# apple/ml-quant

Measured on AMD Instinct MI355X. Metric: images/sec ResNet-18 LS-1w/LS-2a 224x224 eval forward, higher is better.
Workload: dtype fp4 (e2m1, unit block scales) mfma on sign bits: exact integers in the f32 accumulator + f32; 1 GPU; ResNet-18 ImageNet ls-1 weight / ls-2 activation, synthetic 3x224x224, batch 256 per GPU, random-init weights; global_batch=256, parallelism=dp1 (batch-sharded replicas, RCCL all-gather of logits)

## Files before the change

### ml-quant_amd/csrc/lsq_pointwise.hip

```cpp

#include "lsq_common.h"

#ifdef LSQ_PW_SYNCTHREADS
#define PW_BARRIER() __syncthreads()
#else
#define PW_BARRIER() lds_barrier()
#endif
namespace lsq {
namespace {

typedef __attribute__((ext_vector_type(16))) float f32x16;

struct PwArgs {
  const float* x;
  const float* w;
  const float* bias;
  float* y;
  int N, C, H, W, O, Ho, Wo, s;
  long long P;
};

constexpr int kPitch = 68;

__global__ __launch_bounds__(256) void pointwise_conv_kernel(PwArgs a) {
  __shared__ __attribute__((aligned(16))) float ws[64][kPitch];
  __shared__ __attribute__((aligned(16))) float xs[64][kPitch];
  const int tid = threadIdx.x, lane = tid & 63, wid = tid >> 6;
  const unsigned n_ot = (unsigned)a.O >> 6;
  const long long p0 = (long long)(blockIdx.x / n_ot) * 64;
  const int o0 = (int)(blockIdx.x % n_ot) * 64;
  const int HoWo = a.Ho * a.Wo;
  const long long HW = (long long)a.H * a.W;
  const long long sp = min(p0 + lane, a.P - 1);
  const int sn = (int)(sp / HoWo);
  const int sr = (int)(sp - (long long)sn * HoWo);
  const int sho = sr / a.Wo, swo = sr - sho * a.Wo;
  const unsigned xoff = (unsigned)(((long long)sn * a.C + 16 * wid) * HW + (long long)sho * a.s * a.W + swo * a.s);
  const float* __restrict__ xsrc = a.x;
  const unsigned woff = (unsigned)(16 * wid * a.C + lane);
  const float* __restrict__ wsrc = a.w + (long long)o0 * a.C;
  const int mt = wid >> 1, nt = wid & 1;
  const int col = lane & 31, g = lane >> 5;
  f32x16 acc = {};
  float xv[16], wv[16];
#pragma unroll
  for (int i = 0; i < 16; ++i) xv[i] = (xsrc + (long long)i * HW)[xoff];
#pragma unroll
  for (int i = 0; i < 16; ++i) wv[i] = (wsrc + (long long)i * a.C)[woff];
  for (int c0 = 0; c0 < a.C; c0 += 64) {
    __syncthreads();
#pragma unroll
    for (int q = 0; q < 4; ++q)
      *reinterpret_cast<float4*>(&xs[lane][16 * wid + 4 * q]) = make_float4(xv[4 * q], xv[4 * q + 1], xv[4 * q + 2], xv[4 * q + 3]);
#pragma unroll
    for (int i = 0; i < 16; ++i) ws[16 * wid + i][lane] = wv[i];
    __syncthreads();
    if (c0 + 64 < a.C) {
#pragma unroll
      for (int i = 0; i < 16; ++i) xv[i] = (xsrc + (long long)(c0 + 64 + i) * HW)[xoff];
#pragma unroll
      for (int i = 0; i < 16; ++i) wv[i] = (wsrc + (long long)i * a.C + c0 + 64)[woff];
    }
#pragma unroll
    for (int h = 0; h < 2; ++h) {
      float4 af[4], bf[4];
#pragma unroll
      for (int q = 0; q < 4; ++q) {
        af[q] = *reinterpret_cast<const float4*>(&ws[mt * 32 + col][32 * g + 16 * h + 4 * q]);
        bf[q] = *reinterpret_cast<const float4*>(&xs[nt * 32 + col][32 * g + 16 * h + 4 * q]);
      }
#pragma unroll
      for (int q = 0; q < 4; ++q) {
        acc = __builtin_amdgcn_mfma_f32_32x32x2f32(af[q].x, bf[q].x, acc, 0, 0, 0);
        acc = __builtin_amdgcn_mfma_f32_32x32x2f32(af[q].y, bf[q].y, acc, 0, 0, 0);
        acc = __builtin_amdgcn_mfma_f32_32x32x2f32(af[q].z, bf[q].z, acc, 0, 0, 0);
        acc = __builtin_amdgcn_mfma_f32_32x32x2f32(af[q].w, bf[q].w, acc, 0, 0, 0);
      }
    }
  }
  const long long p = p0 + nt * 32 + col;
  const int ob = o0 + mt * 32 + 4 * g;
  float bv[16];
  if (a.bias) {
#pragma unroll
    for (int reg = 0; reg < 16; ++reg) bv[reg] = a.bias[ob + (reg & 3) + 8 * (reg >> 2)];
  } else {
#pragma unroll
    for (int reg = 0; reg < 16; ++reg) bv[reg] = 0.f;
  }
  if (p >= a.P) return;
  const int n = (int)(p / HoWo);
  const int r = (int)(p - (long long)n * HoWo);
  const unsigned yoff = (unsigned)(((long long)n * a.O + ob) * HoWo + r);
#pragma unroll
  for (int reg = 0; reg < 16; ++reg) (a.y + (long long)((reg & 3) + 8 * (reg >> 2)) * HoWo)[yoff] = acc[reg] + bv[reg];
}

typedef float f32x4 __attribute__((ext_vector_type(4)));

template <int NOT, bool PAIRS, bool VEC4>
__global__ __launch_bounds__(256) void pointwise_all_kernel(PwArgs a) {
  __shared__ __attribute__((aligned(16))) float ws[2][64][kPitch];
  __shared__ __attribute__((aligned(16))) float xs[64][kPitch];
  const int tid = threadIdx.x, lane = tid & 63, wid = tid >> 6;
  const long long p0 = (long long)blockIdx.x * 64;
  const int ob = (int)blockIdx.y * (NOT * 64);
  const int HoWo = a.Ho * a.Wo;
  const long long HW = (long long)a.H * a.W;
  const float* __restrict__ xsrc = a.x;
  unsigned xoff;
  if constexpr (PAIRS) {
    const long long sp = min(p0 + 2 * (tid & 31), a.P - 2);
    const int sn = (int)(sp / HoWo);
    const int sr = (int)(sp - (long long)sn * HoWo);
    const int sho = sr / a.Wo, swo = sr - sho * a.Wo;
    xoff = (unsigned)(((long long)sn * a.C + 8 * (tid >> 5)) * HW + (long long)sho * a.s * a.W + swo * a.s);
  } else {
    const long long sp = min(p0 + lane, a.P - 1);
    const int sn = (int)(sp / HoWo);
    const int sr = (int)(sp - (long long)sn * HoWo);
    const int sho = sr / a.Wo, swo = sr - sho * a.Wo;
    xoff = (unsigned)(((long long)sn * a.C + 16 * wid) * HW + (long long)sho * a.s * a.W + swo * a.s);
  }
  const unsigned woff = (unsigned)((tid >> 4) * a.C + 4 * (tid & 15));
  const int mt = wid >> 1, nt = wid & 1;
  const int col = lane & 31, g = lane >> 5;
  f32x16 acc[NOT];
#pragma unroll
  for (int t = 0; t < NOT; ++t)
#pragma unroll
    for (int q = 0; q < 16; ++q) acc[t][q] = 0.f;

  f32x4 xq[8];
  float xv[16];
  auto load_x = [&](int c0) {
    if constexpr (PAIRS) {
#pragma unroll
      for (int i = 0; i < 8; ++i) xq[i] = *reinterpret_cast<const f32x4*>(xsrc + (long long)(c0 + i) * HW + xoff);
    } else {
#pragma unroll
      for (int i = 0; i < 16; ++i) xv[i] = (xsrc + (long long)(c0 + i) * HW)[xoff];
    }
  };
  auto store_x = [&]() {
    if constexpr (PAIRS) {
      const int px = 2 * (tid & 31), cb = 8 * (tid >> 5);
      *reinterpret_cast<float4*>(&xs[px][cb]) = make_float4(xq[0][0], xq[1][0], xq[2][0], xq[3][0]);
      *reinterpret_cast<float4*>(&xs[px][cb + 4]) = make_float4(xq[4][0], xq[5][0], xq[6][0], xq[7][0]);
      *reinterpret_cast<float4*>(&xs[px + 1][cb]) = make_float4(xq[0][2], xq[1][2], xq[2][2], xq[3][2]);
      *reinterpret_cast<float4*>(&xs[px + 1][cb + 4]) = make_float4(xq[4][2], xq[5][2], xq[6][2], xq[7][2]);
    } else {
#pragma unroll
      for (int q = 0; q < 4; ++q)
        *reinterpret_cast<float4*>(&xs[lane][16 * wid + 4 * q]) = make_float4(xv[4 * q], xv[4 * q + 1], xv[4 * q + 2], xv[4 * q + 3]);
    }
  };
  f32x4 wq[4];
  auto load_w = [&](int t, int c0) {
    const float* wsrc = a.w + (long long)(ob + t * 64) * a.C + c0;
#pragma unroll
    for (int k = 0; k < 4; ++k) wq[k] = *reinterpret_cast<const f32x4*>(wsrc + (long long)(16 * k) * a.C + woff);
  };
  auto store_w = [&](int buf) {
#pragma unroll
    for (int k = 0; k < 4; ++k)
      *reinterpret_cast<float4*>(&ws[buf][(tid >> 4) + 16 * k][4 * (tid & 15)]) = make_float4(wq[k][0], wq[k][1], wq[k][2], wq[k][3]);
  };

  const int nchunks = a.C >> 6;
  load_x(0);
  load_w(0, 0);
  int buf = 0;
  for (int cc = 0; cc < nchunks; ++cc) {
    PW_BARRIER();
    store_x();
    if (cc + 1 < nchunks) load_x(64 * (cc + 1));
#pragma unroll
    for (int t = 0; t < NOT; ++t) {
      store_w(buf);
      PW_BARRIER();
      if (t + 1 < NOT) load_w(t + 1, 64 * cc);
      else if (cc + 1 < nchunks) load_w(0, 64 * (cc + 1));
#pragma unroll
      for (int h = 0; h < 2; ++h) {
        float4 af[4], bf[4];
#pragma unroll
        for (int q = 0; q < 4; ++q) {
          af[q] = *reinterpret_cast<const float4*>(&ws[buf][mt * 32 + col][32 * g + 16 * h + 4 * q]);
          bf[q] = *reinterpret_cast<const float4*>(&xs[nt * 32 + col][32 * g + 16 * h + 4 * q]);
        }
#pragma unroll
        for (int q = 0; q < 4; ++q) {
          acc[t] = __builtin_amdgcn_mfma_f32_32x32x2f32(bf[q].x, af[q].x, acc[t], 0, 0, 0);
          acc[t] = __builtin_amdgcn_mfma_f32_32x32x2f32(bf[q].y, af[q].y, acc[t], 0, 0, 0);
          acc[t] = __builtin_amdgcn_mfma_f32_32x32x2f32(bf[q].z, af[q].z, acc[t], 0, 0, 0);
          acc[t] = __builtin_amdgcn_mfma_f32_32x32x2f32(bf[q].w, af[q].w, acc[t], 0, 0, 0);
        }
      }
      buf ^= 1;
    }
  }
#pragma unroll
  for (int t = 0; t < NOT; ++t) {
    const int o = ob + 64 * t + mt * 32 + col;
    const float b = a.bias ? a.bias[o] : 0.f;
#pragma unroll
    for (int rg = 0; rg < 4; ++rg) {
      const long long p = p0 + nt * 32 + 8 * rg + 4 * g;
      if constexpr (VEC4) {
        if (p < a.P) {
          const int n = (int)(p / HoWo);
          const int r = (int)(p - (long long)n * HoWo);
          const f32x4 v = {acc[t][4 * rg] + b, acc[t][4 * rg + 1] + b, acc[t][4 * rg + 2] + b, acc[t][4 * rg + 3] + b};
          *reinterpret_cast<f32x4*>(a.y + ((long long)n * a.O + o) * HoWo + r) = v;
        }
      } else {
#pragma unroll
        for (int k = 0; k < 4; ++k) {
          const long long pk = p + k;
          if (pk < a.P) {
            const int n = (int)(pk / HoWo);
            const int r = (int)(pk - (long long)n * HoWo);
            a.y[((long long)n * a.O + o) * HoWo + r] = acc[t][4 * rg + k] + b;
          }
        }
      }
    }
  }
}

template <int NOT>
void launch_all(const PwArgs& a, dim3 grid, hipStream_t st) {
  const bool vec4 = ((a.Ho * a.Wo) & 3) == 0;
  if (a.s == 2 && (a.Wo & 1) == 0 && a.P >= 2) {
    if (vec4) hipLaunchKernelGGL((pointwise_all_kernel<NOT, true, true>), grid, dim3(256), 0, st, a);
    else hipLaunchKernelGGL((pointwise_all_kernel<NOT, true, false>), grid, dim3(256), 0, st, a);
  } else {
    if (vec4) hipLaunchKernelGGL((pointwise_all_kernel<NOT, false, true>), grid, dim3(256), 0, st, a);
    else hipLaunchKernelGGL((pointwise_all_kernel<NOT, false, false>), grid, dim3(256), 0, st, a);
  }
}

}
}

using namespace lsq;

extern "C" int lsq_pointwise_conv(const float* x, int N, int C, int H, int W, const float* w, const float* bias, int O,
                                  int stride, float* y, void* stream) {
  if (!x || !w || !y) return LSQ_E_NULL;
  if (N <= 0 || C <= 0 || H <= 0 || W <= 0 || O <= 0 || stride <= 0) return LSQ_E_SHAPE;
  if (C % 64 || O % 64) return LSQ_E_UNSUPPORTED;
  if ((long long)N * C * H * W >= (1ll << 30) || (long long)N * O * ((H - 1) / stride + 1) * ((W - 1) / stride + 1) >= (1ll << 30))
    return LSQ_E_UNSUPPORTED;
  PwArgs a = {};
  a.x = x; a.w = w; a.bias = bias; a.y = y;
  a.N = N; a.C = C; a.H = H; a.W = W; a.O = O; a.s = stride;
  a.Ho = (H - 1) / stride + 1;
  a.Wo = (W - 1) / stride + 1;
  a.P = (long long)N * a.Ho * a.Wo;
  const long long blocks = (a.P + 63) / 64;
  if (blocks * (O / 64) > 0x7FFFFFFF) return LSQ_E_SHAPE;
  const int n_ot = O / 64;
  const bool pair_ok = stride != 2 || (a.Wo & 1) || (W & 1) == 0;
  if (n_ot <= 8 && (n_ot & (n_ot - 1)) == 0 && pair_ok) {
    int per_wg = n_ot;
    long long min_wgs = 256;
#ifdef LSQ_TUNE
    if (const char* e = getenv("LSQ_PW_MINWG")) min_wgs = atoll(e);
#endif
    while (per_wg > 1 && blocks * (n_ot / per_wg) < min_wgs) per_wg >>= 1;
    const dim3 grid((unsigned)blocks, (unsigned)(n_ot / per_wg));
    switch (per_wg) {
      case 1: launch_all<1>(a, grid, (hipStream_t)stream); break;
      case 2: launch_all<2>(a, grid, (hipStream_t)stream); break;
      case 4: launch_all<4>(a, grid, (hipStream_t)stream); break;
      default: launch_all<8>(a, grid, (hipStream_t)stream); break;
    }
    return (int)hipGetLastError();
  }
  hipLaunchKernelGGL(pointwise_conv_kernel, dim3((unsigned)(blocks * (O / 64))), dim3(256), 0, (hipStream_t)stream, a);
  return (int)hipGetLastError();
}
```

Measured before the change: 125,000 images/sec.

## Make pointwise conv kernel persistent with double-buffered x and load-balanced tile split

Replaces the one-tile-per-workgroup pointwise (1x1) conv kernel with a persistent kernel. Each workgroup walks a contiguous range of pixel tiles, with the grid sized to 2 workgroups per CU and an optional swizzle for grouping. The x tile is now double-buffered in LDS, weights are prefetched two steps ahead and stay resident when they fit, and output-channel grouping is chosen by a wave-quantization load model. The goal is to cut launch tail and wave-quantization waste, overlap global loads with MFMA work, and drop per-tile index division. The cost is more LDS per workgroup, which lowers occupancy, plus more complex indexing and a hardcoded CU count.

```diff
diff --git a/ml-quant_amd/csrc/lsq_pointwise.hip b/ml-quant_amd/csrc/lsq_pointwise.hip
--- a/ml-quant_amd/csrc/lsq_pointwise.hip
+++ b/ml-quant_amd/csrc/lsq_pointwise.hip
@@ -1,3 +1,6 @@
+
+#include <algorithm>
+#include <type_traits>
 
 #include "lsq_common.h"
 
@@ -97,97 +100,173 @@
 }
 
 typedef float f32x4 __attribute__((ext_vector_type(4)));
-
-template <int NOT, bool PAIRS, bool VEC4>
-__global__ __launch_bounds__(256) void pointwise_all_kernel(PwArgs a) {
+typedef float f32x4u __attribute__((ext_vector_type(4), aligned(4)));
+
+constexpr int kPwCus = 256;
+constexpr int kPwWgsPerCu = 2;
+
+struct PwSplit {
+  unsigned tiles;
+  unsigned ngroups;
+  unsigned base, rem;
+  int swz;
+};
+
+template <int NOT, bool WRES, bool PAIRS>
+__global__ __launch_bounds__(256) void pointwise_persistent_kernel(PwArgs a, PwSplit sp) {
   __shared__ __attribute__((aligned(16))) float ws[2][64][kPitch];
-  __shared__ __attribute__((aligned(16))) float xs[64][kPitch];
+  __shared__ __attribute__((aligned(16))) float xs[2][64][kPitch];
   const int tid = threadIdx.x, lane = tid & 63, wid = tid >> 6;
-  const long long p0 = (long long)blockIdx.x * 64;
-  const int ob = (int)blockIdx.y * (NOT * 64);
-  const int HoWo = a.Ho * a.Wo;
-  const long long HW = (long long)a.H * a.W;
+  unsigned grp, idx;
+  if (sp.swz) {
+    const unsigned k = blockIdx.x >> 3;
+    grp = k % sp.ngroups;
+    idx = (k / sp.ngroups) * 8 + (blockIdx.x & 7);
+  } else {
+    grp = blockIdx.x % sp.ngroups;
+    idx = blockIdx.x / sp.ngroups;
+  }
+  const unsigned tile0 = idx * sp.base + min(idx, sp.rem);
+  const unsigned nu = sp.base + (idx < sp.rem ? 1u : 0u);
+  const int ob = (int)grp * (NOT * 64);
+  const unsigned P = (unsigned)a.P, HoWo = (unsigned)(a.Ho * a.Wo), HW = (unsigned)(a.H * a.W);
+  const int nchunks = a.C >> 6;
   const float* __restrict__ xsrc = a.x;
-  unsigned xoff;
-  if constexpr (PAIRS) {
-    const long long sp = min(p0 + 2 * (tid & 31), a.P - 2);
-    const int sn = (int)(sp / HoWo);
-    const int sr = (int)(sp - (long long)sn * HoWo);
-    const int sho = sr / a.Wo, swo = sr - sho * a.Wo;
-    xoff = (unsigned)(((long long)sn * a.C + 8 * (tid >> 5)) * HW + (long long)sho * a.s * a.W + swo * a.s);
-  } else {
-    const long long sp = min(p0 + lane, a.P - 1);
-    const int sn = (int)(sp / HoWo);
-    const int sr = (int)(sp - (long long)sn * HoWo);
-    const int sho = sr / a.Wo, swo = sr - sho * a.Wo;
-    xoff = (unsigned)(((long long)sn * a.C + 16 * wid) * HW + (long long)sho * a.s * a.W + swo * a.s);
-  }
-  const unsigned woff = (unsigned)((tid >> 4) * a.C + 4 * (tid & 15));
+  auto x_offset = [&](unsigned tile) __attribute__((always_inline)) -> unsigned {
+    const unsigned spx = PAIRS ? min(tile * 64 + 2 * (tid & 31), P - 2) : min(tile * 64 + lane, P - 1);
+    const unsigned sn = spx / HoWo, sr = spx - sn * HoWo;
+    const unsigned sho = sr / (unsigned)a.Wo, swo = sr - sho * (unsigned)a.Wo;
+    return ((sn * a.C + (PAIRS ? 8 * (tid >> 5) : 16 * wid)) * HW + sho * a.s * a.W + swo * a.s) * 4;
+  };
+  f32x4 xq[8];
+  float xv[16];
+  auto load_x = [&](int cc, unsigned xoff) __attribute__((always_inline)) {
+    const char* src = reinterpret_cast<const char*>(xsrc + (long long)(64 * cc) * HW);
+    if constexpr (PAIRS) {
+#pragma unroll
+      for (int i = 0; i < 8; ++i) xq[i] = *reinterpret_cast<const f32x4u*>(src + (long long)i * HW * 4 + xoff);
+    } else {
+#pragma unroll
+      for (int i = 0; i < 16; ++i) xv[i] = *reinterpret_cast<const float*>(src + (long long)i * HW * 4 + xoff);
+    }
+  };
+  auto store_x = [&](int buf) __attribute__((always_inline)) {
+    if constexpr (PAIRS) {
+      const int px = 2 * (tid & 31), cb = 8 * (tid >> 5);
+      *reinterpret_cast<float4*>(&xs[buf][px][cb]) = make_float4(xq[0][0], xq[1][0], xq[2][0], xq[3][0]);
+      *reinterpret_cast<float4*>(&xs[buf][px][cb + 4]) = make_float4(xq[4][0], xq[5][0], xq[6][0], xq[7][0]);
+      *reinterpret_cast<float4*>(&xs[buf][px + 1][cb]) = make_float4(xq[0][2], xq[1][2], xq[2][2], xq[3][2]);
+      *reinterpret_cast<float4*>(&xs[buf][px + 1][cb + 4]) = make_float4(xq[4][2], xq[5][2], xq[6][2], xq[7][2]);
+    } else {
+#pragma unroll
+      for (int q = 0; q < 4; ++q)
+        *reinterpret_cast<float4*>(&xs[buf][lane][16 * wid + 4 * q]) = make_float4(xv[4 * q], xv[4 * q + 1], xv[4 * q + 2], xv[4 * q + 3]);
+    }
+  };
+  const unsigned woff = (unsigned)((tid >> 4) * a.C + 4 * (tid & 15)) * 4;
+  const float* __restrict__ wsrc = a.w + (long long)ob * a.C;
+  f32x4 wq[2][4];
+  auto load_w = [&](f32x4 (&r)[4], int t, int cc) {
+    const char* src = reinterpret_cast<const char*>(wsrc + (long long)(t * 64) * a.C + 64 * cc);
+#pragma unroll
+    for (int k = 0; k < 4; ++k) r[k] = *reinterpret_cast<const f32x4*>(src + (long long)(16 * k) * a.C * 4 + woff);
+  };
+  auto store_w = [&](int buf, const f32x4 (&r)[4]) {
+#pragma unroll
+    for (int k = 0; k < 4; ++k)
+      *reinterpret_cast<float4*>(&ws[buf][(tid >> 4) + 16 * k][4 * (tid & 15)]) = make_float4(r[k][0], r[k][1], r[k][2], r[k][3]);
+  };
   const int mt = wid >> 1, nt = wid & 1;
   const int col = lane & 31, g = lane >> 5;
   f32x16 acc[NOT];
-#pragma unroll
-  for (int t = 0; t < NOT; ++t)
+  float bv[NOT];
+#pragma unroll
+  for (int t = 0; t < NOT; ++t) {
 #pragma unroll
     for (int q = 0; q < 16; ++q) acc[t][q] = 0.f;
-
-  f32x4 xq[8];
-  float xv[16];
-  auto load_x = [&](int c0) {
-    if constexpr (PAIRS) {
-#pragma unroll
-      for (int i = 0; i < 8; ++i) xq[i] = *reinterpret_cast<const f32x4*>(xsrc + (long long)(c0 + i) * HW + xoff);
-    } else {
-#pragma unroll
-      for (int i = 0; i < 16; ++i) xv[i] = (xsrc + (long long)(c0 + i) * HW)[xoff];
-    }
-  };
-  auto store_x = [&]() {
-    if constexpr (PAIRS) {
-      const int px = 2 * (tid & 31), cb = 8 * (tid >> 5);
-      *reinterpret_cast<float4*>(&xs[px][cb]) = make_float4(xq[0][0], xq[1][0], xq[2][0], xq[3][0]);
-      *reinterpret_cast<float4*>(&xs[px][cb + 4]) = make_float4(xq[4][0], xq[5][0], xq[6][0], xq[7][0]);
-      *reinterpret_cast<float4*>(&xs[px + 1][cb]) = make_float4(xq[0][2], xq[1][2], xq[2][2], xq[3][2]);
-      *reinterpret_cast<float4*>(&xs[px + 1][cb + 4]) = make_float4(xq[4][2], xq[5][2], xq[6][2], xq[7][2]);
-    } else {
-#pragma unroll
-      for (int q = 0; q < 4; ++q)
-        *reinterpret_cast<float4*>(&xs[lane][16 * wid + 4 * q]) = make_float4(xv[4 * q], xv[4 * q + 1], xv[4 * q + 2], xv[4 * q + 3]);
-    }
-  };
-  f32x4 wq[4];
-  auto load_w = [&](int t, int c0) {
-    const float* wsrc = a.w + (long long)(ob + t * 64) * a.C + c0;
-#pragma unroll
-    for (int k = 0; k < 4; ++k) wq[k] = *reinterpret_cast<const f32x4*>(wsrc + (long long)(16 * k) * a.C + woff);
-  };
-  auto store_w = [&](int buf) {
-#pragma unroll
-    for (int k = 0; k < 4; ++k)
-      *reinterpret_cast<float4*>(&ws[buf][(tid >> 4) + 16 * k][4 * (tid & 15)]) = make_float4(wq[k][0], wq[k][1], wq[k][2], wq[k][3]);
-  };
-
-  const int nchunks = a.C >> 6;
-  load_x(0);
-  load_w(0, 0);
-  int buf = 0;
-  for (int cc = 0; cc < nchunks; ++cc) {
-    PW_BARRIER();
-    store_x();
-    if (cc + 1 < nchunks) load_x(64 * (cc + 1));
+    bv[t] = a.bias ? a.bias[ob + 64 * t + mt * 32 + col] : 0.f;
+  }
+  const unsigned q64 = 64 / HoWo, r64 = 64 - q64 * HoWo;
+  unsigned pb = tile0 * 64 + nt * 32 + 4 * g;
+  unsigned pn = pb / HoWo, pr = pb - pn * HoWo;
+  char* ydst = reinterpret_cast<char*>(a.y);
+  auto store_tile = [&]() __attribute__((always_inline)) {
+#pragma unroll
+    for (int rg = 0; rg < 4; ++rg) {
+      const unsigned p = pb + 8 * rg;
+      unsigned n = pn, r = pr + 8 * rg;
+      while (r >= HoWo) { r -= HoWo; ++n; }
+      if (p + 3 < P && r + 3 < HoWo) {
+        const unsigned yoff = ((n * a.O + ob + mt * 32 + col) * HoWo + r) * 4;
+#pragma unroll
+        for (int t = 0; t < NOT; ++t) {
+          const f32x4 v = {acc[t][4 * rg] + bv[t], acc[t][4 * rg + 1] + bv[t], acc[t][4 * rg + 2] + bv[t], acc[t][4 * rg + 3] + bv[t]};
+          *reinterpret_cast<f32x4u*>(ydst + (long long)(64 * t) * HoWo * 4 + yoff) = v;
+        }
+      } else {
+#pragma unroll
+        for (int k = 0; k < 4; ++k) {
+          if (p + k < P) {
+            const unsigned yoff = ((n * a.O + ob + mt * 32 + col) * HoWo + r) * 4;
+#pragma unroll
+            for (int t = 0; t < NOT; ++t) *reinterpret_cast<float*>(ydst + (long long)(64 * t) * HoWo * 4 + yoff) = acc[t][4 * rg + k] + bv[t];
+          }
+          if (++r == HoWo) { r = 0; ++n; }
+        }
+      }
+    }
+    pb += 64;
+    pn += q64;
+    pr += r64;
+    if (pr >= HoWo) { pr -= HoWo; ++pn; }
+#pragma unroll
+    for (int t = 0; t < NOT; ++t)
+#pragma unroll
+      for (int q = 0; q < 16; ++q) acc[t][q] = 0.f;
+  };
+
+  unsigned xoff = x_offset(tile0);
+  load_x(0, xoff);
+  load_w(wq[0], 0, 0);
+  load_w(wq[1], 1 % NOT, NOT == 1 ? 1 % nchunks : 0);
+  store_x(0);
+  store_w(0, wq[0]);
+  if constexpr (WRES) store_w(1, wq[1]);
+  PW_BARRIER();
+
+  const unsigned nxc = nu * (unsigned)nchunks;
+  constexpr std::integral_constant<int, 0> kEven;
+  constexpr std::integral_constant<int, 1> kOdd;
+  unsigned j = 0;
+  int cc = 0, xb = 0, wb = 0;
+  auto chunk = [&](auto par0, auto more) __attribute__((always_inline)) {
+    constexpr int PAR = decltype(par0)::value;
+    constexpr bool has_next = decltype(more)::value;
+    int ccn = cc + 1;
+    unsigned xoffn = xoff;
+    if (ccn == nchunks) {
+      ccn = 0;
+      if constexpr (has_next) xoffn = x_offset(tile0 + (j + 1) / (unsigned)nchunks);
+    }
+    if constexpr (has_next) load_x(ccn, xoffn);
+    __builtin_amdgcn_sched_barrier(0);
 #pragma unroll
     for (int t = 0; t < NOT; ++t) {
-      store_w(buf);
-      PW_BARRIER();
-      if (t + 1 < NOT) load_w(t + 1, 64 * cc);
-      else if (cc + 1 < nchunks) load_w(0, 64 * (cc + 1));
+      const int par = (PAR + t) & 1;
+      if constexpr (!WRES) {
+        int c2 = cc + (t + 2) / NOT;
+        if (c2 >= nchunks) c2 -= nchunks;
+        if (c2 >= nchunks) c2 -= nchunks;
+        load_w(wq[par], (t + 2) % NOT, c2);
+        __builtin_amdgcn_sched_barrier(0);
+      }
 #pragma unroll
       for (int h = 0; h < 2; ++h) {
         float4 af[4], bf[4];
 #pragma unroll
         for (int q = 0; q < 4; ++q) {
-          af[q] = *reinterpret_cast<const float4*>(&ws[buf][mt * 32 + col][32 * g + 16 * h + 4 * q]);
-          bf[q] = *reinterpret_cast<const float4*>(&xs[nt * 32 + col][32 * g + 16 * h + 4 * q]);
+          af[q] = *reinterpret_cast<const float4*>(&ws[wb][mt * 32 + col][32 * g + 16 * h + 4 * q]);
+          bf[q] = *reinterpret_cast<const float4*>(&xs[xb][nt * 32 + col][32 * g + 16 * h + 4 * q]);
         }
 #pragma unroll
         for (int q = 0; q < 4; ++q) {
@@ -197,48 +276,50 @@
           acc[t] = __builtin_amdgcn_mfma_f32_32x32x2f32(bf[q].w, af[q].w, acc[t], 0, 0, 0);
         }
       }
-      buf ^= 1;
-    }
-  }
-#pragma unroll
-  for (int t = 0; t < NOT; ++t) {
-    const int o = ob + 64 * t + mt * 32 + col;
-    const float b = a.bias ? a.bias[o] : 0.f;
-#pragma unroll
-    for (int rg = 0; rg < 4; ++rg) {
-      const long long p = p0 + nt * 32 + 8 * rg + 4 * g;
-      if constexpr (VEC4) {
-        if (p < a.P) {
-          const int n = (int)(p / HoWo);
-          const int r = (int)(p - (long long)n * HoWo);
-          const f32x4 v = {acc[t][4 * rg] + b, acc[t][4 * rg + 1] + b, acc[t][4 * rg + 2] + b, acc[t][4 * rg + 3] + b};
-          *reinterpret_cast<f32x4*>(a.y + ((long long)n * a.O + o) * HoWo + r) = v;
-        }
-      } else {
-#pragma unroll
-        for (int k = 0; k < 4; ++k) {
-          const long long pk = p + k;
-          if (pk < a.P) {
-            const int n = (int)(pk / HoWo);
-            const int r = (int)(pk - (long long)n * HoWo);
-            a.y[((long long)n * a.O + o) * HoWo + r] = acc[t][4 * rg + k] + b;
-          }
-        }
-      }
-    }
+      wb ^= 1;
+      __builtin_amdgcn_sched_barrier(0);
+      if constexpr (!WRES) store_w(wb, wq[par ^ 1]);
+      if constexpr (has_next) {
+        if (t == NOT - 1) store_x(xb ^ 1);
+      }
+      if (!WRES || t == NOT - 1) PW_BARRIER();
+    }
+    if (ccn == 0) store_tile();
+    cc = ccn;
+    xoff = xoffn;
+    xb ^= 1;
+    ++j;
+  };
+  if constexpr (NOT == 1 && !WRES) {
+    while (j + 2 < nxc) {
+      chunk(kEven, std::true_type());
+      chunk(kOdd, std::true_type());
+    }
+    if (j + 2 == nxc) {
+      chunk(kEven, std::true_type());
+      chunk(kOdd, std::false_type());
+    } else {
+      chunk(kEven, std::false_type());
+    }
+  } else {
+    while (j + 1 < nxc) chunk(kEven, std::true_type());
+    chunk(kEven, std::false_type());
   }
 }
 
 template <int NOT>
-void launch_all(const PwArgs& a, dim3 grid, hipStream_t st) {
-  const bool vec4 = ((a.Ho * a.Wo) & 3) == 0;
-  if (a.s == 2 && (a.Wo & 1) == 0 && a.P >= 2) {
-    if (vec4) hipLaunchKernelGGL((pointwise_all_kernel<NOT, true, true>), grid, dim3(256), 0, st, a);
-    else hipLaunchKernelGGL((pointwise_all_kernel<NOT, true, false>), grid, dim3(256), 0, st, a);
-  } else {
-    if (vec4) hipLaunchKernelGGL((pointwise_all_kernel<NOT, false, true>), grid, dim3(256), 0, st, a);
-    else hipLaunchKernelGGL((pointwise_all_kernel<NOT, false, false>), grid, dim3(256), 0, st, a);
-  }
+int launch_persistent(const PwArgs& a, const PwSplit& sp, unsigned wgs, hipStream_t st) {
+  const bool pairs = a.s == 2 && (a.Wo & 1) == 0 && a.P >= 2;
+  if constexpr (NOT <= 2) {
+    if ((a.C >> 6) * NOT <= 2) {
+      if (pairs) hipLaunchKernelGGL((pointwise_persistent_kernel<NOT, true, true>), dim3(wgs), dim3(256), 0, st, a, sp);
+      else hipLaunchKernelGGL((pointwise_persistent_kernel<NOT, true, false>), dim3(wgs), dim3(256), 0, st, a, sp);
+      return (int)hipGetLastError();
+    }
+  }
+  if (pairs) hipLaunchKernelGGL((pointwise_persistent_kernel<NOT, false, true>), dim3(wgs), dim3(256), 0, st, a, sp);
+  else hipLaunchKernelGGL((pointwise_persistent_kernel<NOT, false, false>), dim3(wgs), dim3(256), 0, st, a, sp);
+  return (int)hipGetLastError();
 }
 
 }
@@ -264,20 +345,26 @@
   const int n_ot = O / 64;
   const bool pair_ok = stride != 2 || (a.Wo & 1) || (W & 1) == 0;
   if (n_ot <= 8 && (n_ot & (n_ot - 1)) == 0 && pair_ok) {
-    int per_wg = n_ot;
-    long long min_wgs = 256;
-#ifdef LSQ_TUNE
-    if (const char* e = getenv("LSQ_PW_MINWG")) min_wgs = atoll(e);
-#endif
-    while (per_wg > 1 && blocks * (n_ot / per_wg) < min_wgs) per_wg >>= 1;
-    const dim3 grid((unsigned)blocks, (unsigned)(n_ot / per_wg));
+    long long load[5] = {}, best = 0;
+    for (int c = 1; c <= 4 && c <= n_ot; c <<= 1) {
+      load[c] = (blocks * (n_ot / c) + kPwCus - 1) / kPwCus * c;
+      if (c == 1 || load[c] < best) best = load[c];
+    }
+    int per_wg = 1;
+    for (int c = 2; c <= 4 && c <= n_ot; c <<= 1)
+      if (load[c] * 20 <= best * 21) per_wg = c;
+    PwSplit sp = {};
+    sp.tiles = (unsigned)blocks;
+    sp.ngroups = (unsigned)(n_ot / per_wg);
+    const unsigned wpg = (unsigned)std::min<long long>(blocks, kPwCus * kPwWgsPerCu / sp.ngroups);
+    sp.base = sp.tiles / wpg;
+    sp.rem = sp.tiles % wpg;
+    sp.swz = wpg % 8 == 0;
     switch (per_wg) {
-      case 1: launch_all<1>(a, grid, (hipStream_t)stream); break;
-      case 2: launch_all<2>(a, grid, (hipStream_t)stream); break;
-      case 4: launch_all<4>(a, grid, (hipStream_t)stream); break;
-      default: launch_all<8>(a, grid, (hipStream_t)stream); break;
-    }
-    return (int)hipGetLastError();
+      case 1: return launch_persistent<1>(a, sp, wpg * sp.ngroups, (hipStream_t)stream);
+      case 2: return launch_persistent<2>(a, sp, wpg * sp.ngroups, (hipStream_t)stream);
+      default: return launch_persistent<4>(a, sp, wpg * sp.ngroups, (hipStream_t)stream);
+    }
   }
   hipLaunchKernelGGL(pointwise_conv_kernel, dim3((unsigned)(blocks * (O / 64))), dim3(256), 0, (hipStream_t)stream, a);
   return (int)hipGetLastError();
```

Measured after the change: 125,700 images/sec, median of 5. Within noise of the previous version (+0.5%).
